# google/neural-light-transport

Measured on AMD Instinct MI355X. Metric: rendered Mtexels/s at 1024^2 UV (full Model.call forward: U-Net + UV->camera warp); at N > 1: N collective-free replicas of this forward (weak scaling).  The data-parallel TRAIN step with the RCCL gradient all-reduce (BASELINE config 4) is `train_step`: value = Mtexels/s over all ranks, speedup_vs_o, higher is better.
Workload: dtype f32 via 3xbf16 split, 9 exact products, fp32 accumulate (the LDS-tiled encoder convs: fp32 operands as three bf16 terms on v_mfma_f32_16x16x32_bf16, every term product exact in fp32); f32 storage everywhere, every other launch native f32; 1 GPU; BASELINE config 3: dragon_specular relight+view-synth, depth0 16/depth 256, 4 frames/GPU, 1024^2 UV, k=4 obs maps, 512^2 camera warp; frames_per_gpu=4, uv=1024, k=4, cam=512, conv_algo=auto, plan=fused ends, launch=eager, two HIP streams, distinct_batches_rotated=3, launch_tape_replays=0, parallelism=dp1 (frames sharded, no forward collective), world=1, dist_world_size=1, device=cuda:0

## Files before the change

neural-light-transport_amd/csrc/conv_tile3.hip:

```cpp
#include "nlt_common.h"
#include "pack_common.h"

namespace {

typedef __attribute__((ext_vector_type(8))) __bf16 bf16x8;
typedef unsigned short u16;
typedef unsigned int u32x4 __attribute__((ext_vector_type(4)));

constexpr int TH = 8, TW = 16;
constexpr int QS2 = 272, ODD2 = 132;
constexpr int PL = 160;

template <int MODE> struct T3;
template <> struct T3<NLT_CONV_K2S1> { static constexpr int PAIRS = 2, B_UNITS = 153 * 2, B_SLOTS = 6 * PL; };
template <> struct T3<NLT_CONV_K2S2> { static constexpr int PAIRS = 1, B_UNITS = 256 * 2, B_SLOTS = 6 * QS2; };

struct Tile3P {
  const float* src; const u16* packed; const float* bias;
  float* out; float* mean_out;
  int ld, cin, frames, kobs, h, w;
  int oh, ow, cout, ldo, ldm;
  int tiles_y, tiles_x, ncc;
  int act; float alpha;
};

__device__ __forceinline__ int xcd_tile3(int b, int nblocks) {
  return (nblocks & 7) ? b : (b & 7) * (nblocks >> 3) + (b >> 3);
}

__device__ __forceinline__ unsigned cvt_pk_bf16(float a, float b) {
  typedef float f32x2_ __attribute__((ext_vector_type(2)));
  typedef __bf16 bf16x2_ __attribute__((ext_vector_type(2)));
  return __builtin_bit_cast(unsigned, __builtin_convertvector((f32x2_){a, b}, bf16x2_));
}

__device__ __forceinline__ void split2(float a, float b, unsigned& hi, unsigned& mid, unsigned& lo) {
  hi = cvt_pk_bf16(a, b);
  const float ra = a - __uint_as_float(hi << 16), rb = b - __uint_as_float(hi & 0xffff0000u);
  mid = cvt_pk_bf16(ra, rb);
  const float sa = ra - __uint_as_float(mid << 16), sb = rb - __uint_as_float(mid & 0xffff0000u);
  lo = cvt_pk_bf16(sa, sb);
}

__host__ __device__ inline u16 bf16_rne_bits(float f) {
  union { float f; unsigned u; } x; x.f = f;
  x.u += 0x7fffu + ((x.u >> 16) & 1u);
  return (u16)(x.u >> 16);
}
__host__ __device__ inline float bf16_bits_float(u16 b) {
  union { float f; unsigned u; } x; x.u = (unsigned)b << 16;
  return x.f;
}

__global__ void pack_tile3_kernel(const float* __restrict__ wk, int cin, int cout, int tnt, long total, u16* __restrict__ wp) {
  const long idx = (long)blockIdx.x * blockDim.x + threadIdx.x;
  if (idx >= total) return;
  const int e = idx & 7, lane = (idx >> 3) & 63;
  long r = idx >> 9;
  const int term = r % 3; r /= 3;
  const int ct = r % tnt; r /= tnt;
  const int pair = r & 1; r >>= 1;
  const int ncc = cin >> 4;
  const int cc = r % ncc;
  const int g = r / ncc;
  const int kk = lane >> 4, i = lane & 15;
  const int t = pair * 2 + (kk >> 1);
  const int c = cc * 16 + (kk & 1) * 8 + e;
  const int o = (g * tnt + ct) * 16 + i;
  const float v = wk[((long)t * cin + c) * cout + o];
  const u16 hi = bf16_rne_bits(v);
  const float r1 = v - bf16_bits_float(hi);
  const u16 mid = bf16_rne_bits(r1);
  const float r2 = r1 - bf16_bits_float(mid);
  wp[idx] = term == 0 ? hi : (term == 1 ? mid : bf16_rne_bits(r2));
}

template <int MODE, int TNT, int NPROD, int KO>
__global__ __launch_bounds__(256, 2) void conv_tile3_kernel(Tile3P p) {
  using TT = T3<MODE>;
  constexpr int WN = TNT == 4 ? 2 : 1, WM = 4 / WN, RT = TH / WM, CT = 2;
  constexpr int A_SLOTS = TT::PAIRS * TNT * 3 * 64;
  constexpr int NA = (A_SLOTS + 255) / 256, NB = (TT::B_UNITS + 255) / 256;
  __shared__ u32x4 lds[2 * A_SLOTS + 2 * TT::B_SLOTS];

  const int tid = threadIdx.x, lane = tid & 63, wave = tid >> 6;
  const int kk = lane >> 4, j = lane & 15;
  const int wn = wave % WN, wm = wave / WN;
  int tile = xcd_tile3(blockIdx.x, gridDim.x);
  const int tx0 = (tile % p.tiles_x) * TW; tile /= p.tiles_x;
  const int ty0 = (tile % p.tiles_y) * TH;
  const int f = tile / p.tiles_y;
  const int g = blockIdx.y;
  const int spf = (MODE == NLT_CONV_K2S1 ? 1 : 2) * p.ncc;
  const int groups = p.kobs / KO;
  const int total = spf * p.kobs;
  const long in_frame = (long)p.h * p.w;

  int b_lds[NB], b_hf[NB]; long b_tex[NB]; bool b_ok[NB], b_st[NB];
#pragma unroll
  for (int i = 0; i < NB; ++i) {
    const int u = tid + 256 * i;
    const int hf = (u >> 3) & 1, tx = (u >> 4) * 8 + (u & 7);
    b_hf[i] = hf;
    if (MODE == NLT_CONV_K2S1) {
      const int hy = tx / 17, hx = tx % 17;
      const int gy = ty0 + hy, gx = tx0 + hx;
      b_st[i] = tx < 153;
      b_ok[i] = b_st[i] && gy < p.h && gx < p.w;
      b_tex[i] = (long)gy * p.w + gx;
      b_lds[i] = hf * PL + tx;
    } else {
      const int y = tx >> 5, xx = tx & 31;
      const int gy = 2 * (ty0 + y), gx = 2 * tx0 + xx;
      b_st[i] = tx < 256;
      b_ok[i] = b_st[i] && (ty0 + y) < p.oh && gx < p.w;
      b_tex[i] = (long)gy * p.w + gx;
      b_lds[i] = hf * QS2 + (xx & 1) * ODD2 + y * 16 + (xx >> 1);
    }
  }
  constexpr int BPL = MODE == NLT_CONV_K2S1 ? PL : QS2;

  u32x4 ra[NA];
  f32x4 rb[NB][2];
  auto load_a = [&](int s) {
    const int cc = MODE == NLT_CONV_K2S1 ? s : (s >> 1);
    const int a = MODE == NLT_CONV_K2S1 ? 0 : (s & 1);
    const u32x4* ap = reinterpret_cast<const u32x4*>(p.packed) + (((long)g * p.ncc + cc) * 2 + a) * (TNT * 3 * 64);
#pragma unroll
    for (int n = 0; n < NA; ++n) ra[n] = ap[(A_SLOTS % 256 == 0 || tid + 256 * n < A_SLOTS) ? tid + 256 * n : tid];
  };
  auto load_b = [&](int s, int frame) {
    const int cc = MODE == NLT_CONV_K2S1 ? s : (s >> 1);
    const int a = MODE == NLT_CONV_K2S1 ? 0 : (s & 1);
    const float* sp = p.src + ((long)(f * p.kobs + frame) * in_frame + (long)a * p.w) * p.ld + cc * 16;
#pragma unroll
    for (int n = 0; n < NB; ++n) {
      const float* q8 = sp + (b_ok[n] ? b_tex[n] : 0) * p.ld + 8 * b_hf[n];
      const f32x4 v0 = *reinterpret_cast<const f32x4*>(q8), v1 = *reinterpret_cast<const f32x4*>(q8 + 4);
      const f32x4 z = {0.f, 0.f, 0.f, 0.f};
      rb[n][0] = b_ok[n] ? v0 : z;
      rb[n][1] = b_ok[n] ? v1 : z;
    }
  };
  auto store_a = [&](int buf) {
    u32x4* base = lds + buf * A_SLOTS;
#pragma unroll
    for (int n = 0; n < NA; ++n)
      if (A_SLOTS % 256 == 0 || tid + 256 * n < A_SLOTS) base[tid + 256 * n] = ra[n];
  };
  auto store_b = [&](int buf) {
    u32x4* base = lds + 2 * A_SLOTS + buf * TT::B_SLOTS;
#pragma unroll
    for (int n = 0; n < NB; ++n) {
      if (!b_st[n]) continue;
      unsigned hi[4], mid[4], lo[4];
      split2(rb[n][0][0], rb[n][0][1], hi[0], mid[0], lo[0]);
      split2(rb[n][0][2], rb[n][0][3], hi[1], mid[1], lo[1]);
      split2(rb[n][1][0], rb[n][1][1], hi[2], mid[2], lo[2]);
      split2(rb[n][1][2], rb[n][1][3], hi[3], mid[3], lo[3]);
      u32x4* bb = base + b_lds[n];
      bb[0] = (u32x4){hi[0], hi[1], hi[2], hi[3]};
      bb[2 * BPL] = (u32x4){mid[0], mid[1], mid[2], mid[3]};
      bb[4 * BPL] = (u32x4){lo[0], lo[1], lo[2], lo[3]};
    }
  };

  f32x4 acc[KO][RT][CT], mean[RT][CT];
#pragma unroll
  for (int rt = 0; rt < RT; ++rt)
#pragma unroll
    for (int ct = 0; ct < CT; ++ct) {
      mean[rt][ct] = (f32x4){0.f, 0.f, 0.f, 0.f};
#pragma unroll
      for (int io = 0; io < KO; ++io) acc[io][rt][ct] = mean[rt][ct];
    }

  load_a(0);
  load_b(0, 0);
  store_a(0);
  store_b(0);
  __syncthreads();
  int q = 0;
  for (int gi = 0; gi < groups; ++gi) {
    for (int s = 0; s < spf; ++s) {
      const int sa = (gi * spf + s) & 1;
#pragma unroll
      for (int io = 0; io < KO; ++io, ++q) {
        const bool more = q + 1 < total;
        const bool new_slab = io + 1 == KO;
        int ns = s, ngi = gi;
        if (new_slab) { if (++ns == spf) { ns = 0; ++ngi; } }
        if (more) {
          if (new_slab) load_a(ns);
          load_b(ns, ngi * KO + (new_slab ? 0 : io + 1));
        }
        const u32x4* A = lds + sa * A_SLOTS;
        const u32x4* B = lds + 2 * A_SLOTS + (q & 1) * TT::B_SLOTS;
#pragma unroll
        for (int pl = 0; pl < TT::PAIRS; ++pl) {
          bf16x8 bt[3][RT], at[3][CT];
#pragma unroll
          for (int rt = 0; rt < RT; ++rt) {
            const int y = wm * RT + rt;
            const int slot = MODE == NLT_CONV_K2S1 ? (kk & 1) * PL + (y + pl) * 17 + j + (kk >> 1)
                                                   : (kk & 1) * QS2 + (kk >> 1) * ODD2 + y * 16 + j;
#pragma unroll
            for (int t = 0; t < 3; ++t) bt[t][rt] = __builtin_bit_cast(bf16x8, B[t * 2 * BPL + slot]);
          }
#pragma unroll
          for (int ct = 0; ct < CT; ++ct)
#pragma unroll
            for (int t = 0; t < 3; ++t)
              at[t][ct] = __builtin_bit_cast(bf16x8, A[((pl * TNT + wn * CT + ct) * 3 + t) * 64 + lane]);
          constexpr int ORDER9[9][2] = {{2, 2}, {2, 1}, {1, 2}, {2, 0}, {0, 2}, {1, 1}, {1, 0}, {0, 1}, {0, 0}};
#pragma unroll
          for (int pi = 9 - NPROD; pi < 9; ++pi)
#pragma unroll
            for (int rt = 0; rt < RT; ++rt)
#pragma unroll
              for (int ct = 0; ct < CT; ++ct)
                acc[io][rt][ct] = __builtin_amdgcn_mfma_f32_16x16x32_bf16(at[ORDER9[pi][0]][ct], bt[ORDER9[pi][1]][rt], acc[io][rt][ct], 0, 0, 0);
        }
        if (s == spf - 1 && io == KO - 1) {
#pragma unroll
          for (int e = 0; e < KO; ++e) {
            const int i = gi * KO + e;
#pragma unroll
            for (int ct = 0; ct < CT; ++ct) {
              const int oc = (g * TNT + wn * CT + ct) * 16 + 4 * kk;
              const f32x4 bv = *reinterpret_cast<const f32x4*>(p.bias + oc);
#pragma unroll
              for (int rt = 0; rt < RT; ++rt) {
                const int gy = ty0 + wm * RT + rt, gx = tx0 + j;
                f32x4 v = acc[e][rt][ct] + bv;
                if (p.act) {
#pragma unroll
                  for (int c4 = 0; c4 < 4; ++c4) v[c4] = v[c4] > 0.f ? v[c4] : p.alpha * v[c4];
                }
                acc[e][rt][ct] = (f32x4){0.f, 0.f, 0.f, 0.f};
                mean[rt][ct] += v;
                if (gy < p.oh && gx < p.ow) {
                  const long ot = ((long)(f * p.kobs + i) * p.oh + gy) * p.ow + gx;
                  if (p.out) *reinterpret_cast<f32x4*>(p.out + ot * p.ldo + oc) = v;
                  if (p.mean_out && i == p.kobs - 1) {
                    const long mt = ((long)f * p.oh + gy) * p.ow + gx;
                    *reinterpret_cast<f32x4*>(p.mean_out + mt * p.ldm + oc) = mean[rt][ct] * (1.f / (float)p.kobs);
                  }
                }
              }
            }
          }
        }
        if (more) {
          if (new_slab) store_a(sa ^ 1);
          store_b((q + 1) & 1);
        }
        __syncthreads();
      }
    }
  }
}

extern __shared__ u32x4 tile3r_lds[];

template <int MODE, int TNT, int NPROD, int KO, int NWV>
__global__ __launch_bounds__(64 * NWV, 2) void conv_tile3r_kernel(Tile3P p, int ngroups) {
  using TT = T3<MODE>;
  constexpr int NT = 64 * NWV;
  constexpr int WN = TNT == 4 ? 2 : 1, WM = NWV / WN, RT = TH / WM, CT = 2;
  constexpr int A_SLOTS = TT::PAIRS * TNT * 3 * 64;
  constexpr int NB = (TT::B_UNITS + NT - 1) / NT;
  constexpr int BPL = MODE == NLT_CONV_K2S1 ? PL : QS2;
  const int a_group = p.ncc * 2 * TNT * 3 * 64;
  u32x4* const lds_b = tile3r_lds + a_group;

  const int tid = threadIdx.x, lane = tid & 63, wave = tid >> 6;
  const int kk = lane >> 4, j = lane & 15;
  const int wn = wave % WN, wm = wave / WN;
  const int spf = (MODE == NLT_CONV_K2S1 ? 1 : 2) * p.ncc;
  const int groups = p.kobs / KO;
  const long in_frame = (long)p.h * p.w;
  const int tiles = p.frames * p.tiles_y * p.tiles_x;
  const long items = (long)tiles * ngroups;
  const int rank = xcd_tile3(blockIdx.x, gridDim.x);
  int it = (int)(rank * items / gridDim.x);
  const int it_end = (int)((rank + 1) * items / gridDim.x);
  if (it >= it_end) return;

  int b_lds[NB], b_hf[NB]; long b_tex[NB]; bool b_ok[NB], b_st[NB];
#pragma unroll
  for (int i = 0; i < NB; ++i) {
    const int u = tid + NT * i;
    const int hf = (u >> 3) & 1, tx = (u >> 4) * 8 + (u & 7);
    b_hf[i] = hf;
    if (MODE == NLT_CONV_K2S1) {
      b_st[i] = tx < 153;
      b_lds[i] = hf * PL + tx;
    } else {
      const int y = tx >> 5, xx = tx & 31;
      b_st[i] = tx < 256;
      b_lds[i] = hf * QS2 + (xx & 1) * ODD2 + y * 16 + (xx >> 1);
    }
  }
  int ng = 0, nf = 0, nty0 = 0, ntx0 = 0;
  auto geom = [&](int item) {
    ng = item / tiles;
    int t = item - ng * tiles;
    ntx0 = (t % p.tiles_x) * TW; t /= p.tiles_x;
    nty0 = (t % p.tiles_y) * TH;
    nf = t / p.tiles_y;
#pragma unroll
    for (int i = 0; i < NB; ++i) {
      const int u = tid + NT * i;
      const int tx = (u >> 4) * 8 + (u & 7);
      if (MODE == NLT_CONV_K2S1) {
        const int gy = nty0 + tx / 17, gx = ntx0 + tx % 17;
        b_ok[i] = b_st[i] && gy < p.h && gx < p.w;
        b_tex[i] = (long)gy * p.w + gx;
      } else {
        const int y = tx >> 5, xx = tx & 31;
        const int gy = 2 * (nty0 + y), gx = 2 * ntx0 + xx;
        b_ok[i] = b_st[i] && (nty0 + y) < p.oh && gx < p.w;
        b_tex[i] = (long)gy * p.w + gx;
      }
    }
  };

  f32x4 rb[NB][2];
  auto load_b = [&](int s, int frame) {
    const int cc = MODE == NLT_CONV_K2S1 ? s : (s >> 1);
    const int a = MODE == NLT_CONV_K2S1 ? 0 : (s & 1);
    const float* sp = p.src + ((long)(nf * p.kobs + frame) * in_frame + (long)a * p.w) * p.ld + cc * 16;
#pragma unroll
    for (int n = 0; n < NB; ++n) {
      const float* q8 = sp + (b_ok[n] ? b_tex[n] : 0) * p.ld + 8 * b_hf[n];
      const f32x4 v0 = *reinterpret_cast<const f32x4*>(q8), v1 = *reinterpret_cast<const f32x4*>(q8 + 4);
      const f32x4 z = {0.f, 0.f, 0.f, 0.f};
      rb[n][0] = b_ok[n] ? v0 : z;
      rb[n][1] = b_ok[n] ? v1 : z;
    }
  };
  auto store_b = [&](int buf) {
    u32x4* base = lds_b + buf * TT::B_SLOTS;
#pragma unroll
    for (int n = 0; n < NB; ++n) {
      if (!b_st[n]) continue;
      unsigned hi[4], mid[4], lo[4];
      split2(rb[n][0][0], rb[n][0][1], hi[0], mid[0], lo[0]);
      split2(rb[n][0][2], rb[n][0][3], hi[1], mid[1], lo[1]);
      split2(rb[n][1][0], rb[n][1][1], hi[2], mid[2], lo[2]);
      split2(rb[n][1][2], rb[n][1][3], hi[3], mid[3], lo[3]);
      u32x4* bb = base + b_lds[n];
      bb[0] = (u32x4){hi[0], hi[1], hi[2], hi[3]};
      bb[2 * BPL] = (u32x4){mid[0], mid[1], mid[2], mid[3]};
      bb[4 * BPL] = (u32x4){lo[0], lo[1], lo[2], lo[3]};
    }
  };
  auto copy_a = [&](int grp) {
    const u32x4* ap = reinterpret_cast<const u32x4*>(p.packed) + (long)grp * a_group;
    for (int i = tid; i < a_group; i += NT) tile3r_lds[i] = ap[i];
  };

  f32x4 acc[KO][RT][CT], mean[RT][CT];
#pragma unroll
  for (int rt = 0; rt < RT; ++rt)
#pragma unroll
    for (int ct = 0; ct < CT; ++ct) {
      mean[rt][ct] = (f32x4){0.f, 0.f, 0.f, 0.f};
#pragma unroll
      for (int io = 0; io < KO; ++io) acc[io][rt][ct] = mean[rt][ct];
    }

  geom(it);
  load_b(0, 0);
  copy_a(ng);
  store_b(0);
  __syncthreads();
  int q = 0;
  for (; it < it_end; ++it) {
    const int g = ng, f = nf, ty0 = nty0, tx0 = ntx0;
    const bool last_item = it + 1 == it_end;
    for (int gi = 0; gi < groups; ++gi) {
      for (int s = 0; s < spf; ++s) {
#pragma unroll
        for (int io = 0; io < KO; ++io, ++q) {
          const bool new_slab = io + 1 == KO;
          int ns = s, ngi = gi;
          if (new_slab) { if (++ns == spf) { ns = 0; ++ngi; } }
          const bool item_end = ngi == groups;
          if (item_end) {
            ngi = 0;
            if (!last_item) geom(it + 1);
          }
          load_b(ns, ngi * KO + (new_slab ? 0 : io + 1));
          const u32x4* A = tile3r_lds + s * A_SLOTS;
          const u32x4* B = lds_b + (q & 1) * TT::B_SLOTS;
#pragma unroll
          for (int pl = 0; pl < TT::PAIRS; ++pl) {
            bf16x8 bt[3][RT], at[3][CT];
#pragma unroll
            for (int rt = 0; rt < RT; ++rt) {
              const int y = wm * RT + rt;
              const int slot = MODE == NLT_CONV_K2S1 ? (kk & 1) * PL + (y + pl) * 17 + j + (kk >> 1)
                                                     : (kk & 1) * QS2 + (kk >> 1) * ODD2 + y * 16 + j;
#pragma unroll
              for (int t = 0; t < 3; ++t) bt[t][rt] = __builtin_bit_cast(bf16x8, B[t * 2 * BPL + slot]);
            }
#pragma unroll
            for (int ct = 0; ct < CT; ++ct)
#pragma unroll
              for (int t = 0; t < 3; ++t)
                at[t][ct] = __builtin_bit_cast(bf16x8, A[((pl * TNT + wn * CT + ct) * 3 + t) * 64 + lane]);
            constexpr int ORDER9[9][2] = {{2, 2}, {2, 1}, {1, 2}, {2, 0}, {0, 2}, {1, 1}, {1, 0}, {0, 1}, {0, 0}};
#pragma unroll
            for (int pi = 9 - NPROD; pi < 9; ++pi)
#pragma unroll
              for (int rt = 0; rt < RT; ++rt)
#pragma unroll
                for (int ct = 0; ct < CT; ++ct)
                  acc[io][rt][ct] = __builtin_amdgcn_mfma_f32_16x16x32_bf16(at[ORDER9[pi][0]][ct], bt[ORDER9[pi][1]][rt], acc[io][rt][ct], 0, 0, 0);
          }
          if (s == spf - 1 && io == KO - 1) {
#pragma unroll
            for (int e = 0; e < KO; ++e) {
              const int i = gi * KO + e;
#pragma unroll
              for (int ct = 0; ct < CT; ++ct) {
                const int oc = (g * TNT + wn * CT + ct) * 16 + 4 * kk;
                const f32x4 bv = *reinterpret_cast<const f32x4*>(p.bias + oc);
#pragma unroll
                for (int rt = 0; rt < RT; ++rt) {
                  const int gy = ty0 + wm * RT + rt, gx = tx0 + j;
                  f32x4 v = acc[e][rt][ct] + bv;
                  if (p.act) {
#pragma unroll
                    for (int c4 = 0; c4 < 4; ++c4) v[c4] = v[c4] > 0.f ? v[c4] : p.alpha * v[c4];
                  }
                  acc[e][rt][ct] = (f32x4){0.f, 0.f, 0.f, 0.f};
                  mean[rt][ct] += v;
                  if (gy < p.oh && gx < p.ow) {
                    const long ot = ((long)(f * p.kobs + i) * p.oh + gy) * p.ow + gx;
                    if (p.out) *reinterpret_cast<f32x4*>(p.out + ot * p.ldo + oc) = v;
                    if (p.mean_out && i == p.kobs - 1) {
                      const long mt = ((long)f * p.oh + gy) * p.ow + gx;
                      *reinterpret_cast<f32x4*>(p.mean_out + mt * p.ldm + oc) = mean[rt][ct] * (1.f / (float)p.kobs);
                    }
                  }
                  if (i == p.kobs - 1) mean[rt][ct] = (f32x4){0.f, 0.f, 0.f, 0.f};
                }
              }
            }
          }
          if (!(item_end && last_item)) store_b((q + 1) & 1);
          __syncthreads();
        }
      }
    }
    if (!last_item && ng != g) {
      copy_a(ng);
      __syncthreads();
    }
  }
}

constexpr size_t TILE3R_LDS_CU = 160 * 1024;

int tile3r_cus() {
  static const int n = [] {
    int dev = 0, v = 0;
    if (hipGetDevice(&dev) != hipSuccess) return 0;
    if (hipDeviceGetAttribute(&v, hipDeviceAttributeMultiprocessorCount, dev) != hipSuccess) return 0;
    return v;
  }();
  return n;
}

int tile3r_allow_lds(const void* kernel, size_t lds, size_t (&done)[8]) {
  int dev = 0;
  if (lds <= 64 * 1024) return NLT_OK;
  if (hipGetDevice(&dev) != hipSuccess) return NLT_ERR_LAUNCH;
  if (dev >= 0 && dev < 8 && done[dev] >= lds) return NLT_OK;
  if (hipFuncSetAttribute(kernel, hipFuncAttributeMaxDynamicSharedMemorySize, (int)lds) != hipSuccess) return NLT_ERR_LAUNCH;
  if (dev >= 0 && dev < 8) done[dev] = lds;
  return NLT_OK;
}

template <int MODE, int TNT, int NPROD, int KO, int NWV>
int launch3r_k(const Tile3P& p, size_t lds, int nwg, hipStream_t s) {
  auto* k = conv_tile3r_kernel<MODE, TNT, NPROD, KO, NWV>;
  static size_t done[8] = {};
  if (tile3r_allow_lds(reinterpret_cast<const void*>(k), lds, done) != NLT_OK) return NLT_ERR_LAUNCH;
  hipLaunchKernelGGL(k, dim3((unsigned)nwg), dim3(64 * NWV), lds, s, p, p.cout / (16 * TNT));
  NLT_CHECK_LAUNCH();
  return NLT_OK;
}

template <int RT, int NPROD>
__global__ __launch_bounds__(512, 2) void conv_tile3w_kernel(Tile3P p, int ngroups, int tiles_y) {
  constexpr int TNT = 2, CT = 2, NWV = 8;
  constexpr int ROWS = RT + 1, UNITS = ROWS * 17 * 2, NB = (UNITS + 63) / 64;
  constexpr int PLW = (ROWS * 17 + 15) / 16 * 16;
  constexpr int A_SLOTS = 2 * TNT * 3 * 64;
  const int a_group = p.ncc * A_SLOTS;
  const int tid = threadIdx.x, lane = tid & 63, wave = tid >> 6;
  const int kk = lane >> 4, j = lane & 15;
  u32x4* const B = tile3r_lds + a_group + wave * (6 * PLW);
  const long in_frame = (long)p.h * p.w;
  const int tiles = p.frames * tiles_y * p.tiles_x;
  const long items = (long)tiles * ngroups;
  const int rank = xcd_tile3(blockIdx.x, gridDim.x);
  const int it0 = (int)(rank * items / gridDim.x), it1 = (int)((rank + 1) * items / gridDim.x);

  int b_lds[NB], b_hf[NB], b_tx[NB]; long b_tex[NB]; bool b_ok[NB], b_st[NB];
#pragma unroll
  for (int i = 0; i < NB; ++i) {
    const int u = lane + 64 * i;
    b_hf[i] = (u >> 3) & 1;
    b_tx[i] = (u >> 4) * 8 + (u & 7);
    b_st[i] = b_tx[i] < ROWS * 17;
    b_lds[i] = b_hf[i] * PLW + b_tx[i];
  }
  int nf = 0, nty0 = 0, ntx0 = 0;
  auto geom = [&](int t) {
    ntx0 = (t % p.tiles_x) * TW; t /= p.tiles_x;
    nty0 = (t % tiles_y) * RT;
    nf = t / tiles_y;
#pragma unroll
    for (int i = 0; i < NB; ++i) {
      const int gy = nty0 + b_tx[i] / 17, gx = ntx0 + b_tx[i] % 17;
      b_ok[i] = b_st[i] && gy < p.h && gx < p.w;
      b_tex[i] = (long)gy * p.w + gx;
    }
  };
  f32x4 rb[NB][2];
  auto load_b = [&](int cc, int frame) {
    const float* sp = p.src + (long)(nf * p.kobs + frame) * in_frame * p.ld + cc * 16;
#pragma unroll
    for (int n = 0; n < NB; ++n) {
      const float* q8 = sp + (b_ok[n] ? b_tex[n] : 0) * p.ld + 8 * b_hf[n];
      const f32x4 v0 = *reinterpret_cast<const f32x4*>(q8), v1 = *reinterpret_cast<const f32x4*>(q8 + 4);
      const f32x4 z = {0.f, 0.f, 0.f, 0.f};
      rb[n][0] = b_ok[n] ? v0 : z;
      rb[n][1] = b_ok[n] ? v1 : z;
    }
  };
  auto store_b = [&]() {
#pragma unroll
    for (int n = 0; n < NB; ++n) {
      if (!b_st[n]) continue;
      unsigned hi[4], mid[4], lo[4];
      split2(rb[n][0][0], rb[n][0][1], hi[0], mid[0], lo[0]);
      split2(rb[n][0][2], rb[n][0][3], hi[1], mid[1], lo[1]);
      split2(rb[n][1][0], rb[n][1][1], hi[2], mid[2], lo[2]);
      split2(rb[n][1][2], rb[n][1][3], hi[3], mid[3], lo[3]);
      u32x4* bb = B + b_lds[n];
      bb[0] = (u32x4){hi[0], hi[1], hi[2], hi[3]};
      bb[2 * PLW] = (u32x4){mid[0], mid[1], mid[2], mid[3]};
      bb[4 * PLW] = (u32x4){lo[0], lo[1], lo[2], lo[3]};
    }
  };
  auto wave_sync = [&]() {
    __builtin_amdgcn_fence(__ATOMIC_RELEASE, "wavefront");
    __builtin_amdgcn_wave_barrier();
    __builtin_amdgcn_fence(__ATOMIC_ACQUIRE, "wavefront");
  };

  int seg = it0;
  while (seg < it1) {
    const int g = seg / tiles;
    const int seg_end = min(it1, (g + 1) * tiles);
    {
      const u32x4* ap = reinterpret_cast<const u32x4*>(p.packed) + (long)g * a_group;
      for (int i = tid; i < a_group; i += 64 * NWV) tile3r_lds[i] = ap[i];
    }
    __syncthreads();
    int it = seg + wave;
    if (it < seg_end) {
      f32x4 acc[RT][CT], mean[RT][CT];
#pragma unroll
      for (int rt = 0; rt < RT; ++rt)
#pragma unroll
        for (int ct = 0; ct < CT; ++ct) acc[rt][ct] = mean[rt][ct] = (f32x4){0.f, 0.f, 0.f, 0.f};
      geom(it - g * tiles);
      load_b(0, 0);
      store_b();
      wave_sync();
      for (; it < seg_end; it += NWV) {
        const int f = nf, ty0 = nty0, tx0 = ntx0;
        const bool last_item = it + NWV >= seg_end;
        for (int i = 0; i < p.kobs; ++i) {
          for (int s = 0; s < p.ncc; ++s) {
            int ns = s + 1, ni = i;
            if (ns == p.ncc) { ns = 0; ++ni; }
            const bool item_end = ni == p.kobs;
            if (item_end) {
              ni = 0;
              if (!last_item) geom(it + NWV - g * tiles);
            }
            load_b(ns, ni);
            bf16x8 bt[3][ROWS];
#pragma unroll
            for (int r = 0; r < ROWS; ++r)
#pragma unroll
              for (int t = 0; t < 3; ++t)
                bt[t][r] = __builtin_bit_cast(bf16x8, B[t * 2 * PLW + (kk & 1) * PLW + r * 17 + j + (kk >> 1)]);
            wave_sync();
            const u32x4* A = tile3r_lds + s * A_SLOTS;
#pragma unroll
            for (int pl = 0; pl < 2; ++pl) {
              bf16x8 at[3][CT];
#pragma unroll
              for (int ct = 0; ct < CT; ++ct)
#pragma unroll
                for (int t = 0; t < 3; ++t) at[t][ct] = __builtin_bit_cast(bf16x8, A[((pl * TNT + ct) * 3 + t) * 64 + lane]);
              constexpr int ORDER9[9][2] = {{2, 2}, {2, 1}, {1, 2}, {2, 0}, {0, 2}, {1, 1}, {1, 0}, {0, 1}, {0, 0}};
#pragma unroll
              for (int pi = 9 - NPROD; pi < 9; ++pi)
#pragma unroll
                for (int rt = 0; rt < RT; ++rt)
#pragma unroll
                  for (int ct = 0; ct < CT; ++ct)
                    acc[rt][ct] = __builtin_amdgcn_mfma_f32_16x16x32_bf16(at[ORDER9[pi][0]][ct], bt[ORDER9[pi][1]][rt + pl], acc[rt][ct], 0, 0, 0);
            }
            if (!(item_end && last_item)) store_b();
            wave_sync();
            if (s == p.ncc - 1) {
#pragma unroll
              for (int ct = 0; ct < CT; ++ct) {
                const int oc = (g * TNT + ct) * 16 + 4 * kk;
                const f32x4 bv = *reinterpret_cast<const f32x4*>(p.bias + oc);
#pragma unroll
                for (int rt = 0; rt < RT; ++rt) {
                  const int gy = ty0 + rt, gx = tx0 + j;
                  f32x4 v = acc[rt][ct] + bv;
                  if (p.act) {
#pragma unroll
                    for (int c4 = 0; c4 < 4; ++c4) v[c4] = v[c4] > 0.f ? v[c4] : p.alpha * v[c4];
                  }
                  acc[rt][ct] = (f32x4){0.f, 0.f, 0.f, 0.f};
                  mean[rt][ct] += v;
                  if (gy < p.oh && gx < p.ow) {
                    const long ot = ((long)(f * p.kobs + i) * p.oh + gy) * p.ow + gx;
                    if (p.out) *reinterpret_cast<f32x4*>(p.out + ot * p.ldo + oc) = v;
                    if (p.mean_out && i == p.kobs - 1) {
                      const long mt = ((long)f * p.oh + gy) * p.ow + gx;
                      *reinterpret_cast<f32x4*>(p.mean_out + mt * p.ldm + oc) = mean[rt][ct] * (1.f / (float)p.kobs);
                    }
                  }
                  if (i == p.kobs - 1) mean[rt][ct] = (f32x4){0.f, 0.f, 0.f, 0.f};
                }
              }
            }
          }
        }
      }
    }
    seg = seg_end;
    if (seg < it1) __syncthreads();
  }
}

template <int RT>
int launch3w(const Tile3P& p, int nprod, int max_wg, hipStream_t s) {
  constexpr int PLW = ((RT + 1) * 17 + 15) / 16 * 16;
  const size_t lds = (size_t)p.cin * 2 * 384 + 8 * 6 * PLW * sizeof(u32x4);
  if (lds > TILE3R_LDS_CU) return NLT_ERR_UNSUPPORTED;
  const int cus = tile3r_cus();
  if (cus <= 0) return NLT_ERR_LAUNCH;
  const int tiles_y = (p.oh + RT - 1) / RT;
  const long items = (long)p.frames * tiles_y * p.tiles_x * (p.cout / 32);
  long nwg = cus;
  if (max_wg > 0 && nwg > max_wg) nwg = max_wg;
  if (nwg > items) nwg = items;
  auto* k = nprod == 9 ? conv_tile3w_kernel<RT, 9> : conv_tile3w_kernel<RT, 6>;
  static size_t done[2][8] = {};
  if (tile3r_allow_lds(reinterpret_cast<const void*>(k), lds, done[nprod == 9]) != NLT_OK) return NLT_ERR_LAUNCH;
  hipLaunchKernelGGL(k, dim3((unsigned)nwg), dim3(512), lds, s, p, p.cout / 32, tiles_y);
  NLT_CHECK_LAUNCH();
  return NLT_OK;
}

template <int MODE, int TNT, int KO>
int launch3r(const Tile3P& p, int nprod, int max_wg, hipStream_t s) {
  if (nprod != 6 && nprod != 9) return NLT_ERR_UNSUPPORTED;
  if (MODE == NLT_CONV_K2S1 && TNT == 2) {
    int st = launch3w<4>(p, nprod, max_wg, s);
    if (st == NLT_ERR_UNSUPPORTED) st = launch3w<2>(p, nprod, max_wg, s);
    if (st != NLT_ERR_UNSUPPORTED) return st;
  }
  const size_t lds = (size_t)p.cin * TNT * 384 + 2 * T3<MODE>::B_SLOTS * sizeof(u32x4);
  if (lds > TILE3R_LDS_CU) return NLT_ERR_UNSUPPORTED;
  const bool wide = 2 * lds > TILE3R_LDS_CU;
  const int cus = tile3r_cus();
  if (cus <= 0) return NLT_ERR_LAUNCH;
  const long items = (long)p.frames * p.tiles_y * p.tiles_x * (p.cout / (16 * TNT));
  long nwg = (long)cus * (wide ? 1 : 2);
  if (max_wg > 0 && nwg > max_wg) nwg = max_wg;
  if (nwg > items) nwg = items;
  if (items >= (1l << 31)) return NLT_ERR_UNSUPPORTED;
  if (wide) return nprod == 9 ? launch3r_k<MODE, TNT, 9, KO, 8>(p, lds, (int)nwg, s) : launch3r_k<MODE, TNT, 6, KO, 8>(p, lds, (int)nwg, s);
  return nprod == 9 ? launch3r_k<MODE, TNT, 9, KO, 4>(p, lds, (int)nwg, s) : launch3r_k<MODE, TNT, 6, KO, 4>(p, lds, (int)nwg, s);
}

template <int MODE, int TNT, int KO>
int launch3k(const Tile3P& p, int nprod, hipStream_t s, int resident_wg) {
  if (resident_wg >= 0) return launch3r<MODE, TNT, KO>(p, nprod, resident_wg, s);
  const long tiles = (long)p.frames * p.tiles_y * p.tiles_x;
  const dim3 grid((unsigned)tiles, (unsigned)(p.cout / (16 * TNT)));
  if (nprod == 9) hipLaunchKernelGGL((conv_tile3_kernel<MODE, TNT, 9, KO>), grid, dim3(256), 0, s, p);
  else if (nprod == 6) hipLaunchKernelGGL((conv_tile3_kernel<MODE, TNT, 6, KO>), grid, dim3(256), 0, s, p);
  else if (KO > 1) return NLT_ERR_UNSUPPORTED;
  else if (nprod == 3) hipLaunchKernelGGL((conv_tile3_kernel<MODE, TNT, 3, 1>), grid, dim3(256), 0, s, p);
  else hipLaunchKernelGGL((conv_tile3_kernel<MODE, TNT, 1, 1>), grid, dim3(256), 0, s, p);
  NLT_CHECK_LAUNCH();
  return NLT_OK;
}

template <int MODE, int TNT>
int launch3(const Tile3P& p, int nprod, hipStream_t s, int resident_wg) {
  static const int want = [] { const char* e = getenv("NLT_TILE3_KO"); return e ? atoi(e) : 0; }();
  const int cap = want > 0 ? want : (TNT == 2 ? 4 : (MODE == NLT_CONV_K2S1 || resident_wg >= 0 ? 1 : 2));
  if (nprod >= 6) {
    if (TNT == 2 && cap >= 4 && p.kobs % 4 == 0) return launch3k<MODE, TNT, (TNT == 2 ? 4 : 1)>(p, nprod, s, resident_wg);
    if (cap >= 2 && p.kobs % 2 == 0) return launch3k<MODE, TNT, 2>(p, nprod, s, resident_wg);
  }
  return launch3k<MODE, TNT, 1>(p, nprod, s, resident_wg);
}

}

extern "C" long nlt_conv_tile3_packed_elems(int mode, int cin, int cout, int tn) {
  if ((mode != NLT_CONV_K2S1 && mode != NLT_CONV_K2S2) || cin <= 0 || cout <= 0) return -1;
  if ((cin & 15) || (tn != 32 && tn != 64) || cout % tn) return -1;
  return (long)12 * cin * cout;
}

extern "C" int nlt_pack_conv_tile3_weights(int mode, const float* w_keras, int cin, int cout, int tn, unsigned short* packed,
                                           void* stream) {
  const long total = nlt_conv_tile3_packed_elems(mode, cin, cout, tn);
  if (total <= 0) return NLT_ERR_UNSUPPORTED;
  if (!w_keras || !packed || !nlt_aligned16(packed)) return NLT_ERR_BAD_ARG;
  hipLaunchKernelGGL(pack_tile3_kernel, dim3((unsigned)((total + 255) / 256)), dim3(256), 0, static_cast<hipStream_t>(stream),
                     w_keras, cin, cout, tn / 16, total, packed);
  NLT_CHECK_LAUNCH();
  return NLT_OK;
}

static int tile3_forward(int mode, int nprod, const float* src, int ld, int cin, int frames, int kobs, int h, int w,
                         const unsigned short* packed, const float* bias, int cout, int tn,
                         float* out, int ldo, float* mean_out, int ldm, int act, float alpha, int resident_wg, void* stream) {
  if (!src || !packed || !bias || (!out && !mean_out) || (nprod != 1 && nprod != 3 && nprod != 6 && nprod != 9)) return NLT_ERR_BAD_ARG;
  if (frames <= 0 || kobs <= 0 || h <= 0 || w <= 0 || cin <= 0 || cout <= 0) return NLT_ERR_BAD_ARG;
  if (nlt_conv_tile3_packed_elems(mode, cin, cout, tn) <= 0) return NLT_ERR_UNSUPPORTED;
  if (mode == NLT_CONV_K2S2 && ((h | w) & 1)) return NLT_ERR_UNSUPPORTED;
  if (ld < cin || (ld & 3) || (out && (ldo < cout || (ldo & 3))) || (mean_out && (ldm < cout || (ldm & 3)))) return NLT_ERR_BAD_ARG;
  if (!nlt_aligned16(src) || !nlt_aligned16(packed) || !nlt_aligned16(bias) || (out && !nlt_aligned16(out)) ||
      (mean_out && !nlt_aligned16(mean_out))) return NLT_ERR_BAD_ARG;
  if ((long long)frames * kobs * h * w * (long long)(ld > ldo ? ld : ldo) >= (1ll << 31)) return NLT_ERR_UNSUPPORTED;
  Tile3P p;
  p.src = src; p.packed = packed; p.bias = bias; p.out = out; p.mean_out = mean_out;
  p.ld = ld; p.cin = cin; p.frames = frames; p.kobs = kobs; p.h = h; p.w = w;
  p.oh = mode == NLT_CONV_K2S2 ? h / 2 : h; p.ow = mode == NLT_CONV_K2S2 ? w / 2 : w;
  p.cout = cout; p.ldo = ldo; p.ldm = ldm; p.ncc = cin / 16; p.act = act; p.alpha = alpha;
  p.tiles_y = (p.oh + TH - 1) / TH; p.tiles_x = (p.ow + TW - 1) / TW;
  hipStream_t s = static_cast<hipStream_t>(stream);
  if (mode == NLT_CONV_K2S1)
    return tn == 64 ? launch3<NLT_CONV_K2S1, 4>(p, nprod, s, resident_wg) : launch3<NLT_CONV_K2S1, 2>(p, nprod, s, resident_wg);
  return tn == 64 ? launch3<NLT_CONV_K2S2, 4>(p, nprod, s, resident_wg) : launch3<NLT_CONV_K2S2, 2>(p, nprod, s, resident_wg);
}

extern "C" int nlt_conv_tile3_forward(int mode, int nprod, const float* src, int ld, int cin, int frames, int kobs, int h, int w,
                                      const unsigned short* packed, const float* bias, int cout, int tn,
                                      float* out, int ldo, float* mean_out, int ldm, int act, float alpha, void* stream) {
  return tile3_forward(mode, nprod, src, ld, cin, frames, kobs, h, w, packed, bias, cout, tn, out, ldo, mean_out, ldm, act, alpha,
                       -1, stream);
}

extern "C" int nlt_conv_tile3r_forward(int mode, int nprod, const float* src, int ld, int cin, int frames, int kobs, int h, int w,
                                       const unsigned short* packed, const float* bias, int cout, int tn,
                                       float* out, int ldo, float* mean_out, int ldm, int act, float alpha, int max_workgroups,
                                       void* stream) {
  if (max_workgroups < 0) return NLT_ERR_BAD_ARG;
  return tile3_forward(mode, nprod, src, ld, cin, frames, kobs, h, w, packed, bias, cout, tn, out, ldo, mean_out, ldm, act, alpha,
                       max_workgroups, stream);
}
```

Measured before the change: 3621 Mtexels/s.

## Add resident stride-2 conv kernel streaming B fragments directly from global into registers

Adds a persistent 512-thread kernel for the stride-2 2x2 encoder convs. Each workgroup keeps only the packed weights for one output-channel group in LDS, and each wave loads its input pixels from global memory straight into registers. The 3xbf16 split of those inputs is interleaved with the MFMA term products, and the next slice is prefetched while the current one computes. Each wave handles RT output rows, with RT chosen at 4, 2 or 1 from the available work. This drops the LDS staging of the B operand and its barriers. The trade-off is uncoalesced-ish global loads and higher register pressure.

```diff
diff --git a/neural-light-transport_amd/csrc/conv_tile3.hip b/neural-light-transport_amd/csrc/conv_tile3.hip
--- a/neural-light-transport_amd/csrc/conv_tile3.hip
+++ b/neural-light-transport_amd/csrc/conv_tile3.hip
@@ -680,6 +680,192 @@
   return NLT_OK;
 }
 
+template <int RT, int TNT, int NPROD>
+__global__ __launch_bounds__(512, 2) void conv_tile3s2_kernel(Tile3P p, int ngroups, int tiles_y) {
+  constexpr int NWV = 8;
+  constexpr int A_SLOTS = TNT * 3 * 64;
+  static_assert(9 - RT >= 9 - NPROD, "a row is split beside each of the last RT term products");
+  const int spf = 2 * p.ncc;
+  const int a_group = spf * A_SLOTS;
+  const int tid = threadIdx.x, lane = tid & 63;
+  const int wave = __builtin_amdgcn_readfirstlane(tid >> 6);
+  const int kk = lane >> 4, j = lane & 15;
+  const long in_frame = (long)p.h * p.w;
+  const int tiles = p.frames * tiles_y * p.tiles_x;
+  const long items = (long)tiles * ngroups;
+  const int rank = xcd_tile3(blockIdx.x, gridDim.x);
+  const int it0 = (int)(rank * items / gridDim.x), it1 = (int)((rank + 1) * items / gridDim.x);
+
+  int nf = 0, nty0 = 0, ntx0 = 0;
+  long b_off[RT];
+  auto geom = [&](int t) {
+    ntx0 = (t % p.tiles_x) * TW; t /= p.tiles_x;
+    nty0 = (t % tiles_y) * RT;
+    nf = t / tiles_y;
+#pragma unroll
+    for (int r = 0; r < RT; ++r) {
+      const bool ok = nty0 + r < p.oh && ntx0 + j < p.ow;
+      b_off[r] = (ok ? ((long)2 * r * p.w + 2 * j + (kk >> 1)) * p.ld : 0) + (kk & 1) * 8;
+    }
+  };
+  f32x4 rb[RT][2];
+  auto load_b = [&](int s, int frame) {
+    const float* sp = p.src + ((long)(nf * p.kobs + frame) * in_frame + (long)(2 * nty0 + (s & 1)) * p.w + 2 * ntx0) * p.ld + (s >> 1) * 16;
+#pragma unroll
+    for (int r = 0; r < RT; ++r) {
+      const float* q8 = sp + b_off[r];
+      rb[r][0] = *reinterpret_cast<const f32x4*>(q8);
+      rb[r][1] = *reinterpret_cast<const f32x4*>(q8 + 4);
+    }
+  };
+  bf16x8 bt[3][RT], btn[3][RT];
+  auto split_b = [&](int r) {
+    unsigned hi[4], mid[4], lo[4];
+    split2(rb[r][0][0], rb[r][0][1], hi[0], mid[0], lo[0]);
+    split2(rb[r][0][2], rb[r][0][3], hi[1], mid[1], lo[1]);
+    split2(rb[r][1][0], rb[r][1][1], hi[2], mid[2], lo[2]);
+    split2(rb[r][1][2], rb[r][1][3], hi[3], mid[3], lo[3]);
+    u32x4 h4 = {hi[0], hi[1], hi[2], hi[3]}, m4 = {mid[0], mid[1], mid[2], mid[3]}, l4 = {lo[0], lo[1], lo[2], lo[3]};
+    asm volatile("" : "+v"(h4), "+v"(m4), "+v"(l4));
+    btn[0][r] = __builtin_bit_cast(bf16x8, h4);
+    btn[1][r] = __builtin_bit_cast(bf16x8, m4);
+    btn[2][r] = __builtin_bit_cast(bf16x8, l4);
+  };
+  auto next_b = [&]() {
+#pragma unroll
+    for (int r = 0; r < RT; ++r)
+#pragma unroll
+      for (int t = 0; t < 3; ++t) bt[t][r] = btn[t][r];
+  };
+
+  int seg = it0;
+  while (seg < it1) {
+    const int g = seg / tiles;
+    const int seg_end = min(it1, (g + 1) * tiles);
+    int it = seg + wave;
+    if (it < seg_end) {
+      geom(it - g * tiles);
+      load_b(0, 0);
+    }
+    {
+      const u32x4* ap = reinterpret_cast<const u32x4*>(p.packed) + (long)g * a_group;
+      for (int i = tid; i < a_group; i += 64 * NWV) tile3r_lds[i] = ap[i];
+    }
+    __syncthreads();
+    if (it < seg_end) {
+      f32x4 acc[RT][TNT], mean[RT][TNT];
+#pragma unroll
+      for (int rt = 0; rt < RT; ++rt)
+#pragma unroll
+        for (int ct = 0; ct < TNT; ++ct) acc[rt][ct] = mean[rt][ct] = (f32x4){0.f, 0.f, 0.f, 0.f};
+#pragma unroll
+      for (int r = 0; r < RT; ++r) split_b(r);
+      next_b();
+      for (; it < seg_end; it += NWV) {
+        const int f = nf, ty0 = nty0, tx0 = ntx0;
+        const bool last_item = it + NWV >= seg_end;
+        for (int i = 0; i < p.kobs; ++i) {
+          for (int s = 0; s < spf; ++s) {
+            int ns = s + 1, ni = i;
+            if (ns == spf) { ns = 0; ++ni; }
+            if (ni == p.kobs) {
+              ni = 0;
+              if (!last_item) geom(it + NWV - g * tiles);
+            }
+            load_b(ns, ni);
+            __builtin_amdgcn_sched_barrier(0);
+            const u32x4* A = tile3r_lds + s * A_SLOTS;
+            bf16x8 at[3][TNT];
+#pragma unroll
+            for (int ct = 0; ct < TNT; ++ct)
+#pragma unroll
+              for (int t = 0; t < 3; ++t) at[t][ct] = __builtin_bit_cast(bf16x8, A[(ct * 3 + t) * 64 + lane]);
+            constexpr int ORDER9[9][2] = {{2, 2}, {2, 1}, {1, 2}, {2, 0}, {0, 2}, {1, 1}, {1, 0}, {0, 1}, {0, 0}};
+#pragma unroll
+            for (int pi = 9 - NPROD; pi < 9; ++pi) {
+              if (pi >= 9 - RT) {
+                __builtin_amdgcn_sched_barrier(0);
+                split_b(pi - (9 - RT));
+              }
+#pragma unroll
+              for (int rt = 0; rt < RT; ++rt)
+#pragma unroll
+                for (int ct = 0; ct < TNT; ++ct)
+                  acc[rt][ct] = __builtin_amdgcn_mfma_f32_16x16x32_bf16(at[ORDER9[pi][0]][ct], bt[ORDER9[pi][1]][rt], acc[rt][ct], 0, 0, 0);
+            }
+            __builtin_amdgcn_sched_barrier(0);
+            next_b();
+            if (s == spf - 1) {
+#pragma unroll
+              for (int ct = 0; ct < TNT; ++ct) {
+                const int oc = (g * TNT + ct) * 16 + 4 * kk;
+                const f32x4 bv = *reinterpret_cast<const f32x4*>(p.bias + oc);
+#pragma unroll
+                for (int rt = 0; rt < RT; ++rt) {
+                  const int gy = ty0 + rt, gx = tx0 + j;
+                  f32x4 v = acc[rt][ct] + bv;
+                  if (p.act) {
+#pragma unroll
+                    for (int c4 = 0; c4 < 4; ++c4) v[c4] = v[c4] > 0.f ? v[c4] : p.alpha * v[c4];
+                  }
+                  acc[rt][ct] = (f32x4){0.f, 0.f, 0.f, 0.f};
+                  mean[rt][ct] += v;
+                  if (gy < p.oh && gx < p.ow) {
+                    const long ot = ((long)(f * p.kobs + i) * p.oh + gy) * p.ow + gx;
+                    if (p.out) *reinterpret_cast<f32x4*>(p.out + ot * p.ldo + oc) = v;
+                    if (p.mean_out && i == p.kobs - 1) {
+                      const long mt = ((long)f * p.oh + gy) * p.ow + gx;
+                      *reinterpret_cast<f32x4*>(p.mean_out + mt * p.ldm + oc) = mean[rt][ct] * (1.f / (float)p.kobs);
+                    }
+                  }
+                  if (i == p.kobs - 1) mean[rt][ct] = (f32x4){0.f, 0.f, 0.f, 0.f};
+                }
+              }
+            }
+          }
+        }
+      }
+    }
+    seg = seg_end;
+    if (seg < it1) __syncthreads();
+  }
+}
+
+template <int RT, int TNT, int NPROD>
+int launch3s2_k(const Tile3P& p, size_t lds, int nwg, int tiles_y, hipStream_t s) {
+  auto* k = conv_tile3s2_kernel<RT, TNT, NPROD>;
+  static size_t done[8] = {};
+  if (tile3r_allow_lds(reinterpret_cast<const void*>(k), lds, done) != NLT_OK) return NLT_ERR_LAUNCH;
+  hipLaunchKernelGGL(k, dim3((unsigned)nwg), dim3(512), lds, s, p, p.cout / (16 * TNT), tiles_y);
+  NLT_CHECK_LAUNCH();
+  return NLT_OK;
+}
+
+template <int RT, int TNT>
+int launch3s2_rt(const Tile3P& p, int nprod, size_t lds, long nwg, long per_row, hipStream_t s) {
+  const int tiles_y = (p.oh + RT - 1) / RT;
+  const long items = per_row * tiles_y;
+  if (items >= (1l << 31)) return NLT_ERR_UNSUPPORTED;
+  if (nwg > items) nwg = items;
+  return nprod == 9 ? launch3s2_k<RT, TNT, 9>(p, lds, (int)nwg, tiles_y, s) : launch3s2_k<RT, TNT, 6>(p, lds, (int)nwg, tiles_y, s);
+}
+
+template <int TNT>
+int launch3s2(const Tile3P& p, int nprod, int max_wg, hipStream_t s) {
+  if (nprod != 6 && nprod != 9) return NLT_ERR_UNSUPPORTED;
+  if ((size_t)p.cin * TNT * 384 + 2 * T3<NLT_CONV_K2S2>::B_SLOTS * sizeof(u32x4) > TILE3R_LDS_CU) return NLT_ERR_UNSUPPORTED;
+  const size_t lds = (size_t)p.cin * TNT * 384;
+  const int cus = tile3r_cus();
+  if (cus <= 0) return NLT_ERR_LAUNCH;
+  long nwg = cus;
+  if (max_wg > 0 && nwg > max_wg) nwg = max_wg;
+  const long per_row = (long)p.frames * p.tiles_x * (p.cout / (16 * TNT));
+  if constexpr (TNT == 2)
+    if (per_row * ((p.oh + 3) / 4) >= 8 * nwg) return launch3s2_rt<4, TNT>(p, nprod, lds, nwg, per_row, s);
+  if (per_row * ((p.oh + 1) / 2) >= 8 * nwg) return launch3s2_rt<2, TNT>(p, nprod, lds, nwg, per_row, s);
+  return launch3s2_rt<1, TNT>(p, nprod, lds, nwg, per_row, s);
+}
+
 template <int MODE, int TNT, int KO>
 int launch3r(const Tile3P& p, int nprod, int max_wg, hipStream_t s) {
   if (nprod != 6 && nprod != 9) return NLT_ERR_UNSUPPORTED;
@@ -704,7 +890,10 @@
 
 template <int MODE, int TNT, int KO>
 int launch3k(const Tile3P& p, int nprod, hipStream_t s, int resident_wg) {
-  if (resident_wg >= 0) return launch3r<MODE, TNT, KO>(p, nprod, resident_wg, s);
+  if (resident_wg >= 0) {
+    if constexpr (MODE == NLT_CONV_K2S2) return launch3s2<TNT>(p, nprod, resident_wg, s);
+    else return launch3r<MODE, TNT, KO>(p, nprod, resident_wg, s);
+  }
   const long tiles = (long)p.frames * p.tiles_y * p.tiles_x;
   const dim3 grid((unsigned)tiles, (unsigned)(p.cout / (16 * TNT)));
   if (nprod == 9) hipLaunchKernelGGL((conv_tile3_kernel<MODE, TNT, 9, KO>), grid, dim3(256), 0, s, p);
```

Result: slower. 3573 Mtexels/s (-1.3%).
